# Bebra777228/PolGen-RVC

Hardware: AMD Instinct MI355X
Metric: real-time-factor (audio-sec/wall-sec) per GPU, 30s@16kHz RMVPE->48kHz (higher is better)
Workload: dtype f32 (conv products as 3 fp16 MFMAs of a hi/lo split, fp32 accumulate; fp32 elsewhere)

## Files before the change

include/rvcx.h:

```cpp
#ifndef RVCX_H
#define RVCX_H
#include <stdint.h>

#ifdef __cplusplus
extern "C" {
#endif

typedef struct rvcx_ctx rvcx_ctx;

typedef struct {
  const char* name;
  const void* data;
  int32_t dtype;
  int32_t ndim;
  int64_t shape[4];
} rvcx_tensor;

typedef struct {
  int32_t inter_channels, hidden_channels, filter_channels, n_heads, n_layers, kernel_size;
  int32_t n_resblocks;
  int32_t res_kernels[4];
  int32_t res_dilations[4][3];
  int32_t n_ups;
  int32_t up_rates[6], up_kernels[6];
// ... 364 lines not shown
                      int32_t* coarse, float* f0);
int rvcx_op_conv1d(rvcx_ctx*, const float* x, const float* w, const float* bias, const float* res,
                   float* y, int B, int Cin, int Tin, int Cout, int K, int stride, int dil,
                   int pad_left, int Tout, int groups, int pre_lrelu, float pre_slope, int act,
                   float act_slope, const int32_t* lens_in, const int32_t* lens_out);
int rvcx_op_resblock_pair(rvcx_ctx*, const float* x, const float* w1, const float* b1, const float* w2,
                          const float* b2, float* y, int B, int C, int T, int K, int dil, float slope, int fused,
                          const int32_t* lens);
int rvcx_op_resblock3(rvcx_ctx*, const float* x, const float* w1, const float* b1, const float* w2, const float* b2,
                      float* y, int B, int C, int T, const int32_t* dils, float slope, const int32_t* lens);
int rvcx_bench_resblock_pair(rvcx_ctx*, int B, int C, int T, int K, int dil, int fused, int iters,
                             float* ms_per_launch);
int rvcx_bench_conv1d(rvcx_ctx*, int B, int Cin, int Tin, int Cout, int K, int stride, int dil, int groups,
                      int iters, float* ms_per_launch);
int rvcx_conv_override(int tile, int variant, int splitk);
int rvcx_fx_stretch_override(int chunk_frames, int segment_frames);
int rvcx_op_convtranspose1d(rvcx_ctx*, const float* x, const float* w, const float* bias, float* y,
                            int B, int Cin, int Tin, int Cout, int K, int stride, int pad,
                            int pre_lrelu, float pre_slope);
int rvcx_op_conv2d3x3(rvcx_ctx*, const float* x, const float* w, const float* bias, const float* res,
                      float* y, int B, int Cin, int H, int W, int Cout, int act);
int rvcx_op_convblock2d(rvcx_ctx*, const float* x, const float* w1, const float* b1, const float* w2, const float* b2,
                        const float* wsc, const float* bsc, float* y, int B, int Cin, int Cout, int H, int W,
                        const int32_t* rows);
int rvcx_op_convtranspose2d(rvcx_ctx*, const float* x, const float* w, const float* bias, float* y,
                            int B, int Cin, int H, int W, int Cout, int act);
int rvcx_op_attention(rvcx_ctx*, const float* q, const float* k, const float* v, float* out, int B,
                      int H, int D, int T, float scale, const float* emb_rel_k,
                      const float* emb_rel_v, int window, const int32_t* lens);
int rvcx_op_gemm_tm(rvcx_ctx*, const float* x_cf, const float* w, const float* bias, const float* res_tm, int B, int T,
// ... 39 lines not shown
```

polgen-rvc_amd/_lib.py:

```python
from __future__ import annotations

import ctypes as C
import os
import threading
import types
from typing import Optional, Sequence

import numpy as np

_HERE = os.path.dirname(os.path.abspath(__file__))
LIB_PATH = os.environ.get("RVCX_LIBRARY") or os.path.join(_HERE, "librvcx.so")


class RvcxError(RuntimeError):
    pass


class Tensor(C.Structure):
    _fields_ = [("name", C.c_char_p), ("data", C.c_void_p), ("dtype", C.c_int32),
                ("ndim", C.c_int32), ("shape", C.c_int64 * 4)]


class SynthCfg(C.Structure):
    _fields_ = [("inter_channels", C.c_int32), ("hidden_channels", C.c_int32),
# ... 98 lines not shown
    k = min(Lx, Lb)
    fin = np.sin(0.5 * np.pi * np.arange(Lx) / max(Lx - 1, 1)) ** 2
    out[:k] = y[d:d + k] * fin[:k] + b[:k] * (1.0 - fin[:k])
    return out, y[d + Lb:d + Lb + Lx].copy(), d, scores, mags


_lib = None

SYMBOLS = [
    "rvcx_create", "rvcx_destroy", "rvcx_last_error", "rvcx_version", "rvcx_load_hubert",
    "rvcx_load_rmvpe", "rvcx_index_exhaustive", "rvcx_load_crepe", "rvcx_crepe_frames", "rvcx_crepe_predict", "rvcx_op_crepe_decode", "rvcx_get_f0_crepe_x", "rvcx_load_fcpe", "rvcx_fcpe_f0", "rvcx_fcpe_frames", "rvcx_get_f0_fcpe_x", "rvcx_op_fcpe_post", "rvcx_load_synth", "rvcx_unload_synth", "rvcx_load_index", "rvcx_load_index_ivf",
    "rvcx_weights_regions", "rvcx_weights_adopt", "rvcx_weights_clone", "rvcx_rmvpe_f0", "rvcx_rmvpe_frames", "rvcx_rmvpe_mel", "rvcx_synth_infer_taps", "rvcx_hubert_features",
    "rvcx_hubert_frames", "rvcx_synth_infer", "rvcx_synth_infer_window", "rvcx_synth_dec_rf", "rvcx_synth_upp", "rvcx_index_blend",
    "rvcx_out_len", "rvcx_convert_batch", "rvcx_convert_batch_f64", "rvcx_micro_batch", "rvcx_bucket_length", "rvcx_last_micro_batches", "rvcx_last_cuts", "rvcx_noise_len",
    "rvcx_get_f0", "rvcx_get_f0_x", "rvcx_vc", "rvcx_vc_frames", "rvcx_last_timing",
    "rvcx_flop_counter", "rvcx_fp32_reruns", "rvcx_mem_info", "rvcx_conv_profile", "rvcx_conv_profile_csv", "rvcx_stream", "rvcx_op_conv1d", "rvcx_op_resblock_pair", "rvcx_bench_resblock_pair", "rvcx_bench_conv1d", "rvcx_conv_override", "rvcx_op_convtranspose1d",
    "rvcx_op_conv2d3x3", "rvcx_op_convblock2d", "rvcx_op_convtranspose2d", "rvcx_op_attention", "rvcx_op_layernorm_c",
    "rvcx_op_bigru", "rvcx_op_highpass", "rvcx_highpass_exact", "rvcx_convert_batch_ex", "rvcx_get_f0_x_ex", "rvcx_fp32_layers", "rvcx_fp32_pinned",
    "rvcx_gru_fallbacks", "rvcx_gru_publish_probe", "rvcx_debug_inject", "rvcx_f0_file_track", "rvcx_op_gemm_tm", "rvcx_op_layernorm_tm",
    "rvcx_resample_len", "rvcx_resample_f64", "rvcx_resample_f64_kind", "rvcx_bench_gemm", "rvcx_device_info",
    "rvcx_convert_submit", "rvcx_convert_wait", "rvcx_convert_poll", "rvcx_convert_inflight", "rvcx_ticket_lead_ms",
    "rvcx_synth_infer_head", "rvcx_op_sola", "rvcx_stream_open", "rvcx_stream_step", "rvcx_stream_reset", "rvcx_stream_close",
    "rvcx_stream_out_len", "rvcx_stream_noise_len", "rvcx_stream_frames",
    "rvcx_stream_open_io", "rvcx_stream_in_len", "rvcx_stream_delays", "rvcx_stream_resample_delay", "rvcx_stream_last_taps",
    "rvcx_stream_set", "rvcx_op_stream_resample",
    "rvcx_stream_open_fx", "rvcx_stream_out_channels", "rvcx_stream_set_fx", "rvcx_stream_last_fx_ms", "rvcx_op_stream_fx",
    "rvcx_fx_reverb_host",
    "rvcx_fx_chain", "rvcx_op_fx_highpass", "rvcx_op_fx_compressor", "rvcx_op_fx_gate", "rvcx_op_fx_reverb", "rvcx_op_fx_shelf",
    "rvcx_op_fx_chorus", "rvcx_op_fx_mix", "rvcx_fx_chunk", "rvcx_fx_last_passes", "rvcx_fx_cte", "rvcx_fx_delay",
    "rvcx_fx_coeffs", "rvcx_fx_highpass_host", "rvcx_fx_biquad_host", "rvcx_fx_follower_host", "rvcx_fx_compressor_host",
    "rvcx_fx_gate_host", "rvcx_fx_comb_host", "rvcx_fx_allpass_host", "rvcx_fx_chorus_host", "rvcx_fx_mix_host",
# ... 1029 lines not shown
        self._ck(lib().rvcx_op_resblock3(self._h, _p(x), _p(w1), _p(b1), _p(w2), _p(b2), _p(y), B, Cc, T, _p(d, C.c_int32),
                                         C.c_float(slope), _p(li, C.c_int32)), "op_resblock3")
        return y

    def bench_resblock_pair(self, B, Cc, T, K, dil=1, fused=True, iters=10):
        ms = C.c_float(0)
        self._ck(lib().rvcx_bench_resblock_pair(self._h, B, Cc, T, K, dil, 1 if fused else 0, iters, C.byref(ms)),
                 "bench_resblock_pair")
        return ms.value, 4.0 * B * Cc * Cc * K * T / (ms.value * 1e-3) / 1e12

    @staticmethod
    def conv_override(tile=-1, variant=-1, splitk=-1):
        if lib().rvcx_conv_override(tile, variant, splitk) != 0:
            raise RvcxError("conv_override: " + (lib().rvcx_last_error(None) or b"").decode())

    def bench_conv1d(self, B, Cin, Tin, Cout, K, stride=1, dil=1, groups=1, iters=10):
        ms = C.c_float(0)
        self._ck(lib().rvcx_bench_conv1d(self._h, B, Cin, Tin, Cout, K, stride, dil, groups, iters, C.byref(ms)),
                 "bench_conv1d")
        pad = (K * dil - dil) // 2
        Tout = (Tin + 2 * pad - dil * (K - 1) - 1) // stride + 1
        flops = 2.0 * B * Cout * Tout * K * (Cin // groups)
        return ms.value, flops / (ms.value * 1e-3) / 1e12

    def convtranspose1d(self, x, w, bias=None, stride=1, pad=0, pre_lrelu=None):
        x, w = f32(x), f32(w)
        B, Cin, Tin = x.shape
        _, Cout, K = w.shape
        Tout = (Tin - 1) * stride - 2 * pad + K
        y = np.empty((B, Cout, Tout), np.float32)
# ... 1065 lines not shown
```

polgen-rvc_amd/csrc/api_ops.hip:

```cpp
#include "api_internal.h"
#include "h3_device.h"

using namespace rvcx;
using namespace rvcx::api;

static void to_host(Ctx& c, float* h, const float* d, size_t n) {
  RVCX_HIP(hipMemcpyAsync(h, d, n * sizeof(float), hipMemcpyDeviceToHost, c.stream));
  RVCX_HIP(hipStreamSynchronize(c.stream));
}
#define TEMP_REGION(C) WeightRegion tmp_region_; RegionScope tmp_scope_(*(C), tmp_region_)

extern "C" {

int rvcx_op_conv1d(rvcx_ctx* ctx, const float* x, const float* w, const float* bias, const float* res,
                   float* y, int B, int Cin, int Tin, int Cout, int K, int stride, int dil,
                   int pad_left, int Tout, int groups, int pre_lrelu, float pre_slope, int act,
                   float act_slope, const int32_t* lens_in, const int32_t* lens_out) {
  API_BEGIN(ctx)
  TEMP_REGION(C);
  size_t nx = (size_t)B * Cin * Tin, ny = (size_t)B * Cout * Tout;
  C->arena.reserve((nx + 2 * ny) * 4 + (64 << 20));
  C->arena.reset();
  ConvW L = make_conv(*C, w, bias, Cout, Cin / groups, K, groups, true);
  float* dx = to_dev(*C, x, nx);
// ... 219 lines not shown
  *ms_per_launch = ms / iters;
  (void)hipEventDestroy(e0);
  (void)hipEventDestroy(e1);
  C->arena.reset();
  API_END
}

int rvcx_conv_override(int tile, int variant, int splitk) {
  REQUIRE_DEBUG(nullptr, "rvcx_conv_override")
  rvcx::g_conv_override.tile = tile;
  rvcx::g_conv_override.variant = variant;
  rvcx::g_conv_override.splitk = splitk;
  return 0;
}

int rvcx_bench_conv1d(rvcx_ctx* ctx, int B, int Cin, int Tin, int Cout, int K, int stride, int dil, int groups,
                      int iters, float* ms_per_launch) {
  REQUIRE_DEBUG(ctx, "rvcx_bench_conv1d")
  API_BEGIN(ctx)
  TEMP_REGION(C);
  const int pad = (K * dil - dil) / 2;
  const int Tout = (Tin + 2 * pad - dil * (K - 1) - 1) / stride + 1;
  size_t nx = (size_t)B * Cin * Tin, ny = (size_t)B * Cout * Tout;
  C->arena.reserve((nx + 2 * ny) * 4 + (64 << 20));
  C->arena.reset();
  std::vector<float> w((size_t)Cout * (Cin / groups) * K), bias((size_t)Cout, 0.1f);
  for (size_t i = 0; i < w.size(); ++i) w[i] = (float)((i * 2654435761u) % 2001) / 1000.f - 1.f;
  ConvW L = make_conv(*C, w.data(), bias.data(), Cout, Cin / groups, K, groups, true);
  float* dx = C->arena.alloc<float>(nx);
  float* dy = C->arena.alloc<float>(ny);
// ... 652 lines not shown
```

polgen-rvc_amd/csrc/conv.h:

```cpp
#pragma once
#include "common.h"

namespace rvcx {

enum Act { ACT_NONE = 0, ACT_LRELU = 1, ACT_RELU = 2, ACT_GELU = 3, ACT_TANH = 4, ACT_SIGMOID = 5 };
enum OutMode { OUT_NORMAL = 0, OUT_SHUF1D = 1, OUT_SHUF2D = 2, OUT_TRANSPOSED = 3 };
enum Acc2 { ACC2_NONE = 0, ACC2_SET = 1, ACC2_ADD = 2, ACC2_ADD_DIV = 3 };

struct ConvArgs {
  const float* x = nullptr;
  const float* w = nullptr;
  const void* w_h3 = nullptr;
  const void* x_split = nullptr;
  void* y_split = nullptr;
  const float* bias = nullptr;
  const float* res = nullptr;
  float* y = nullptr;
  float* y2 = nullptr;
  const int* lens_in = nullptr;
  const int* lens_out = nullptr;
  int B = 1;
  int Cin_g = 0, Cin_gp = 0, Cout_g = 0, Cout_gp = 0, groups = 1;
  int Tin = 0;
  int Nout = 0;
// ... 102 lines not shown
struct ConvProfile {
  static constexpr int kMaxTiles = 72;
  long launches[kMaxTiles] = {0};
  double flops[kMaxTiles] = {0};
  double ms[kMaxTiles] = {0};
  int bm[kMaxTiles] = {0}, bn[kMaxTiles] = {0}, halo[kMaxTiles] = {0};
};
void conv_profile_begin();
void conv_profile_end(ConvProfile* out);
const char* conv_profile_csv();
void conv_init();
void launch_conv(ConvArgs a, hipStream_t stream);
int launch_conv_fast(ConvArgs& a, hipStream_t stream);
void conv_fast_describe(ConvProfile* p);
int launch_conv_h3(ConvArgs& a, int halo, int off_min, hipStream_t stream);
bool convt_thin_ok(const ConvArgs& a);
void launch_convt_thin(const ConvArgs& a, hipStream_t stream);
void convt_thin_init();
constexpr int kConvtThinSlot = 61;
bool conv3_thin_ok(const ConvArgs& a);
void launch_conv3_thin(const ConvArgs& a, hipStream_t stream);
constexpr int kConv3ThinSlot = 59;
bool conv_deep_ok(const ConvArgs& a);
void launch_conv_deep(const ConvArgs& a, hipStream_t stream);
constexpr int kConvDeepSlot = 63;
bool conv_h3_enabled();
bool conv_h3_configured();
bool conv_h3_split_ok(const ConvArgs& a);
void launch_splitk_finish(const ConvArgs& a, hipStream_t stream);
void conv_h3_describe(ConvProfile* p);
// ... 20 lines not shown
```

polgen-rvc_amd/csrc/conv.hip:

```cpp
#include "conv.h"
#include "conv_device.h"
#include "gemm.h"

#include <algorithm>
#include <cmath>

namespace rvcx {

template <int BM, int BN, int WR, int WC>
__global__ __launch_bounds__(256) void conv_mfma_kernel(const ConvArgs a) {
  constexpr int WM = BM / (32 * WR), WN = BN / (32 * WC);
  static_assert(WR * WC == 4 && WM >= 1 && WN >= 1, "bad tile");
  extern __shared__ float smem[];
  float* As = smem;
  float* Bs = smem + a.kk_chunk * a.ci_chunk * BM;

  const int tid = threadIdx.x, lane = tid & 63, wave = tid >> 6;
  const int wr = wave / WC, wc = wave % WC;
  const int i = lane & 31, h = lane >> 5;
  const int b = blockIdx.z;
  const int mt_per_g = (a.Cout_gp + BM - 1) / BM;
  const int g = blockIdx.y / mt_per_g, mt = blockIdx.y % mt_per_g;
  const int co0 = mt * BM;
  const int n0 = blockIdx.x * BN;
// ... 136 lines not shown
namespace {
struct ProfRec {
  hipEvent_t a, b;
  int tile;
  double flops;
  int cin, cout, k, nout, stride, B;
};
bool g_prof_on = false;
std::vector<ProfRec> g_prof;
}

void conv_profile_begin() {
  g_prof.clear();
  g_prof_on = true;
}

static std::string g_prof_csv;
const char* conv_profile_csv() { return g_prof_csv.c_str(); }

void conv_profile_end(ConvProfile* out) {
  g_prof_on = false;
  g_prof_csv = "tile,B,cin,cout,k,stride,nout,gflop,ms,tflops\n";
  for (int t = 0; t < kNumTiles; ++t) {
    out->bm[t] = kTiles[t].bm;
    out->bn[t] = kTiles[t].bn;
    out->halo[t] = -1;
  }
  conv_fast_describe(out);
  conv_h3_describe(out);
  resblock_pair_describe(out);
// ... 175 lines not shown
```

polgen-rvc_amd/csrc/conv_fast.hip:

```cpp
#include <cmath>
#include <cstdlib>

#include "conv.h"
#include "conv_device.h"

#ifdef RVCX_ABLATION
#define RVCX_DBG(a, bit) ((a).dbg & (bit))
#else
#define RVCX_DBG(a, bit) 0
#endif

namespace rvcx {

struct BufRsrc {
#if defined(__HIP_DEVICE_COMPILE__)
  __amdgpu_buffer_rsrc_t r;
#endif
};
constexpr int kBufOob = 0x7ffffff0;
__device__ __forceinline__ BufRsrc make_rsrc(const float* base, int bytes) {
  BufRsrc b;
#if defined(__HIP_DEVICE_COMPILE__)
  b.r = __builtin_amdgcn_make_buffer_rsrc(const_cast<float*>(base), 0, bytes, 0x00020000);
#endif
// ... 450 lines not shown
  p->bn[kConvDeepSlot] = 320;
  p->halo[kConvDeepSlot] = 300003;
  for (int t = 0; t < kNumFast; ++t) {
    const int s = 8 + t;
    p->bm[s] = kFast[t].bm;
    p->bn[s] = kFast[t].bn;
    p->halo[s] = kFast[t].cic == 32 ? 100000 : (kFast[t].halo < 0 ? 200000 : kFast[t].halo * 10);
  }
}

void launch_splitk_finish(const ConvArgs& a, hipStream_t stream) {
  const long total = (long)a.B * a.Cout_g * a.Nout;
  const long work = (((long)a.Cout_g * a.Nout) & 3) == 0 ? cdiv64(total, 4) : total;
  hipLaunchKernelGGL(conv_splitk_finish_kernel, dim3((unsigned)std::min<long>(cdiv64(work, 256), 4096)), dim3(256), 0,
                     stream, a);
}

int launch_conv_fast(ConvArgs& a, hipStream_t stream) {
  if (a.Cin_g == 1 && a.groups == 1 && a.ksize <= kCin1MaxK && a.kw >= 1 && a.ksize % a.kw == 0) {
    hipLaunchKernelGGL(conv_cin1_kernel, dim3(cdiv(a.Nout, 256), cdiv(a.Cout_g, 16), a.B), dim3(256), 0, stream, a);
    RVCX_HIP(hipGetLastError());
    return 7;
  }
  if (convt_thin_ok(a)) {
    launch_convt_thin(a, stream);
    return kConvtThinSlot;
  }
  RVCX_CHECK(!a.nz_har || a.out_mode == OUT_SHUF1D, "conv: a fused noise conv needs a polyphase ConvTranspose1d launch");
  if (conv_cout1_ok(a)) {
    static const bool on = !getenv("RVCX_COUT1") || atoi(getenv("RVCX_COUT1")) != 0;
// ... 108 lines not shown
```

polgen-rvc_amd/csrc/conv_h3.hip:

```cpp
#include <algorithm>
#include <cmath>
#include <cstdlib>

#include "conv.h"
#include "conv_device.h"
#include "h3_device.h"

#ifdef RVCX_ABLATION
#define H3_DBG(a, bit) ((a).dbg & (bit))
#else
#define H3_DBG(a, bit) 0
#endif

namespace rvcx {

template <int BM, int BN, int WR, int WC, int KKT, int HALO, int STRIDE, bool LIN, bool XS = false>
__global__ __launch_bounds__(256, ((LIN && BM * BN >= 8192) || BN >= 512) ? 2 : 3) void conv_h3_kernel(const ConvArgs a) {
  constexpr int WM = BM / (32 * WR), WN = BN / (32 * WC);
  constexpr int WROW = LIN ? BN : BN * STRIDE + HALO;
  constexpr int NBTILE = LIN ? KKT : 1;
  constexpr int A_ELEMS = KKT * 2 * 2 * BM;
  constexpr int NA = (A_ELEMS + 255) / 256;
  constexpr int B_TASKS = NBTILE * 2 * WROW;
  constexpr int NBT = (B_TASKS + 255) / 256;
// ... 310 lines not shown
  if (a.groups != 1 || a.ksize == 1 || a.out_mode != OUT_NORMAL) return false;
  if (a.stride != 1 && !(a.stride == 2 && a.kw == a.ksize)) return false;
  if (a.Cin_g % 16 != 0 || a.Cout_g % 16 != 0 || a.Cin_g != a.Cin_gp) return false;
  {
    int lo = 1 << 30, hi = -(1 << 30);
    for (int kk = 0; kk < a.ksize; ++kk) {
      lo = std::min(lo, conv_tap_off(a, kk));
      hi = std::max(hi, conv_tap_off(a, kk));
    }
    if (hi - lo > 320) return false;
  }
  if ((long)a.Cin_gp * a.x_cs * 4 >= kH3Oob || (long)a.Cout_g * a.y_cs * 4 >= kH3Oob) return false;
  return true;
}

int launch_conv_h3(ConvArgs& a, int halo, int off_min, hipStream_t stream) {
  const bool split = a.x_split || a.y_split;
  RVCX_CHECK(!split || conv_h3_split_ok(a), "conv_h3: pre-split activations on a launch that cannot take them");
  if (!a.w_h3 || !conv_h3_enabled()) return -1;
  if (a.Cin_gp % 16 != 0 || (a.stride != 1 && !(a.stride == 2 && a.kw == a.ksize))) return -1;
  if (a.groups != 1 && (split || a.ksize == 1 || a.stride != 1 || a.out_mode != OUT_NORMAL || a.Cin_g != a.Cin_gp)) return -1;
  if ((long)a.Cin_gp * a.x_cs * 4 >= kH3Oob || (long)a.ksize * a.Cin_gp * a.Cout_gp * 4 >= kH3Oob) return -1;
  const bool lin = a.ksize == 1 && a.stride == 1;
  const int nchunk = a.Cin_gp / 16;
  const long cap_item = a.part_cap_item > 0 ? a.part_cap_item : a.part_cap;
  static const bool wide3x3 = getenv("RVCX_WIDE3X3") && atoi(getenv("RVCX_WIDE3X3")) != 0;
  auto select = [&](int Bsel, int forcedS, int* tile_out, int* s_out) {
    int best = -1, S = 1;
    double best_t = 1e300;
    for (int t = 0; t < kNumH3; ++t) {
      const H3Cfg& F = kH3[t];
// ... 24 lines not shown
    *tile_out = best;
    *s_out = S;
  };
  int best = -1, S = 1;
  select(1, 0, &best, &S);
  static const int tile2_mask = getenv("RVCX_TILE2_MASK") ? atoi(getenv("RVCX_TILE2_MASK")) : 255;
  const int cls = (a.out_mode != OUT_NORMAL) ? 8 : (lin ? 2 : (halo > 64 ? 1 : 4));
  int cls2 = cls;
  if (a.x_split || a.y_split) cls2 |= 16;
  const bool tile_for_batch = (tile2_mask & cls) && (!(cls2 & 16) || (tile2_mask & 16));
  if (best >= 0 && a.B > 1 && tile_for_batch) {
    int b2 = -1, s2 = 1;
    select(a.B, S, &b2, &s2);
    if (b2 >= 0 && s2 == S) best = b2;
  }
  if (best < 0) return -1;
  const H3Cfg& F = kH3[best];
  a.off_min = off_min;
  a.wrow = halo;
  a.splitk = S;
  {
    static int dbg = -1;
    if (dbg < 0) dbg = getenv("RVCX_CONV_DBG") ? atoi(getenv("RVCX_CONV_DBG")) : 0;
    a.dbg = dbg;
  }
  dim3 grid(cdiv(a.Nout, F.bn), cdiv(a.Cout_gp, F.bm), a.B * a.groups * S);
  {
    static const bool log = getenv("RVCX_CONV_LOG") != nullptr;
    if (log)
      fprintf(stderr, "h3 tile %d (%dx%d halo %d) S %d grid %u %u %u B %d Cin %d Cout %d k %d Nout %d xs %d ys %d\n", best,
// ... 11 lines not shown
```

polgen-rvc_amd/csrc/ctx.h:

```cpp
#pragma once
#include <memory>

#include "common.h"
#include "conv.h"
#include "gemm.h"

namespace rvcx {

struct SynthModel;
struct RmvpeModel;
struct FcpeModel;
struct CrepeModel;
struct HubertModel;
struct IndexData;

class WeightRegion {
 public:
  static constexpr size_t kChunkBytes = (size_t)32 << 20;
  static constexpr int kMaxFlags = 4096;
  static constexpr size_t kHeaderBytes = kMaxFlags;
  WeightRegion() {
    flags_.reset(new uint8_t[kMaxFlags]);
    std::memset(flags_.get(), 0, kMaxFlags);
  }
// ... 224 lines not shown
  }
  void gemm_on(GemmArgs a, hipStream_t s) {
    const double f = 2.0 * (double)a.rows * a.cout * a.cin;
    flops += f;
    a.ovf = dev_err;
    a.seq = ++launch_seq;
    {
      const int si = (s == stream2) ? 1 : (s == aux[0] ? 2 : (s == aux[1] ? 3 : 0));
      if (!splitk_buf[si]) RVCX_HIP(hipMalloc(&splitk_buf[si], kSplitKFloats * splitk_items * sizeof(float)));
      a.part = splitk_buf[si];
      a.part_cap = kSplitKFloats * splitk_items;
    }
    conv_launch_gemm(a, f, s);
  }
  void conv(const ConvArgs& a) { conv_on(a, stream); }
  void conv_on(ConvArgs a, hipStream_t s) {
    flops += conv_flops(a);
    const int si = (s == stream2) ? 1 : (s == aux[0] ? 2 : (s == aux[1] ? 3 : 0));
    if (!splitk_buf[si]) RVCX_HIP(hipMalloc(&splitk_buf[si], kSplitKFloats * splitk_items * sizeof(float)));
    a.part = splitk_buf[si];
    a.part_cap = kSplitKFloats * splitk_items;
    a.part_cap_item = kSplitKFloats;
    a.ovf = dev_err;
    a.seq = ++launch_seq;
    launch_conv(a, s);
  }
};

struct RegionScope {
  Ctx& c;
  WeightRegion* prev;
  RegionScope(Ctx& cc, WeightRegion& r) : c(cc), prev(cc.slab.cur_) { cc.slab.cur_ = &r; }
  ~RegionScope() { c.slab.cur_ = prev; }
};

struct ConvW {
  const float* w = nullptr;
// ... 56 lines not shown
```

polgen-rvc_amd/csrc/layers.h:

```cpp
#pragma once
#include "ctx.h"

namespace rvcx {

inline ConvArgs conv1d_args(const ConvW& w, const float* x, float* y, int B, int Tin, int Tout,
                            int stride = 1, int dil = 1, int pad = 0) {
  ConvArgs a;
  conv_set_weights(a, w);
  a.x = x;
  a.y = y;
  a.B = B;
  a.Tin = Tin;
  a.Nout = Tout;
  a.stride = stride;
  a.dil = dil;
  a.pad = pad;
  a.x_bs = (long)w.cin * Tin;
  a.x_cs = Tin;
  a.y_bs = (long)w.cout * Tout;
  a.y_cs = Tout;
  return a;
}

inline void conv_set_res(ConvArgs& a, const float* res, int C, int T) {
// ... 75 lines not shown
  a.rowpitch = Wp;
  a.dil = 1;
  a.pad = 0;
  a.stride = 1;
  a.x_bs = (long)L.w.cin * H * Wp;
  a.x_cs = H * Wp;
  a.y_bs = (long)L.cout_real * 2 * H * Wpo;
  a.y_cs = 2 * H * Wpo;
  a.out_mode = OUT_SHUF2D;
  a.sh_cout = L.cout_real;
  a.wp_in = Wp;
  a.wp_out = Wpo;
  return a;
}

ConvT1dW make_convT1d(Ctx& c, const float* w, const float* bias, int cin, int cout, int k, int s, int p);
ConvT2dW make_convT2d(Ctx& c, const float* w, const float* scale, const float* shift, int cin, int cout);

}
```

polgen-rvc_amd/csrc/synth.hip:

```cpp
#include <algorithm>
#include <cmath>
#include <cstdlib>

#include "models.h"
#include "ops.h"

namespace rvcx {

std::vector<float> wn_weight(const TensorTable& t, const std::string& p, int dim) {
  if (t.has(p + ".weight")) return t.f32(p + ".weight");
  std::string gn = p + ".parametrizations.weight.original0", vn = p + ".parametrizations.weight.original1";
  if (!t.has(gn)) {
    gn = p + ".weight_g";
    vn = p + ".weight_v";
  }
  std::vector<float> g = t.f32(gn), v = t.f32(vn);
  const auto shp = t.shape(vn);
  RVCX_CHECK(shp.size() == 3, "weight-norm tensor must be 3-D: " + p);
  const int64_t d0 = shp[0], d1 = shp[1], d2 = shp[2];
  std::vector<float> w(v.size());
  if (dim == 0) {
    RVCX_CHECK((int64_t)g.size() == d0, "weight_g shape: " + p);
    for (int64_t a = 0; a < d0; ++a) {
      double ss = 0.0;
// ... 317 lines not shown
    launch_copy_strided(z + head, z2, B * inter, Tk, T, Tk, s);
    std::swap(z, z2);
  }
  float* g = A.alloc<float>((size_t)B * gin);
  for (int b = 0; b < B; ++b)
    RVCX_HIP(hipMemcpyAsync(g + (size_t)b * gin, m.emb_g + (size_t)sidv[b] * gin, gin * sizeof(float),
                            hipMemcpyDeviceToDevice, s));
  {
    float* h = att;
    float* xin = qkv;
    float* acts = tmp;
    float* rs = hbuf;
    RVCX_CHECK(filt >= 2 * hid, "buffer reuse assumes filter_channels >= 2*hidden");
    float* wout = A.alloc<float>((size_t)B * hid * T);
    float* mbuf = A.alloc<float>((size_t)B * half * T);
    float* gc = A.alloc<float>((size_t)B * 6 * hid);
    for (int f = 3; f >= 0; --f) {
      const auto& F = m.flows[f];
      launch_flip_channels(z, z2, B, inter, Tk, s);
      std::swap(z, z2);
      ConvArgs a = conv1d_args(F.pre, z, h, B, Tk, Tk);
      a.x_bs = (long)inter * Tk;
      a.lens_out = lens;
      c.conv(a);
      a = conv1d_args(F.cond, g, gc, B, 1, 1);
      c.conv(a);
      for (int i = 0; i < 3; ++i) {
        a = conv1d_args(F.in_l[i], h, xin, B, Tk, Tk, 1, 1, (F.in_l[i].k - 1) / 2);
        a.lens_in = lens;
        a.lens_out = lens;
        c.conv(a);
        launch_wn_gate(xin, gc, i * 2 * hid, 6 * hid, acts, B, hid, Tk, s);
        a = conv1d_args(F.rs_l[i], acts, rs, B, Tk, Tk);
        a.lens_out = lens;
        c.conv(a);
        launch_wn_res_skip(h, wout, rs, B, hid, Tk, i == 2, i == 0, lens, s);
      }
      a = conv1d_args(F.post, wout, mbuf, B, Tk, Tk);
      a.lens_out = lens;
      c.conv(a);
      launch_coupling_sub(z, mbuf, B, half, Tk, lens, s);
    }
  }
  if (io.z_out)
    RVCX_HIP(hipMemcpyAsync(io.z_out, z, (size_t)B * inter * Tk * sizeof(float), hipMemcpyDeviceToDevice, s));
  tm.mark(2);
  if (io.ev_decoder) RVCX_HIP(hipEventRecord(io.ev_decoder, s));

  if (!c.serial) RVCX_HIP(hipStreamWaitEvent(s, c.ev_src[1], 0));
  static const int dec_batch_env = getenv("RVCX_DEC_BATCH") ? std::max(1, atoi(getenv("RVCX_DEC_BATCH"))) : 8;
  bool equal_lens = true;
  if (io.lens_host)
    for (int b = 1; b < B; ++b) equal_lens &= io.lens_host[b] == io.lens_host[0];
  const int dec_batch = equal_lens ? dec_batch_env : 1;
  const int C0 = cf.up_initial_channel;
// ... 203 lines not shown
```

Before: 1233.

## Fuse each flow coupling layer into a single LDS-resident kernel with halo

Adds a fused kernel that runs an entire residual-coupling flow layer (pre conv, three WN dilated convs with gating, res/skip convs, post conv and coupling subtraction) for a time window plus halo in LDS, using the hi/lo fp16 MFMA scheme. This replaces about 15 launches per flow and their global round trips with one launch per flow. The channel flip is folded into the indexing, and the cond convs for all four flows are hoisted ahead of the loop. The cost is recomputing halo columns and heavy LDS use, which may limit occupancy. The fused path is on by default when h3 is enabled, profiling is off and the shapes fit.

```diff
diff --git a/include/rvcx.h b/include/rvcx.h
--- a/include/rvcx.h
+++ b/include/rvcx.h
@@ -402,6 +402,8 @@
 int rvcx_bench_conv1d(rvcx_ctx*, int B, int Cin, int Tin, int Cout, int K, int stride, int dil, int groups,
                       int iters, float* ms_per_launch);
 int rvcx_conv_override(int tile, int variant, int splitk);
+int rvcx_flow_fuse_override(int mode, int width);
+int64_t rvcx_flow_fused_launches(void);
 int rvcx_fx_stretch_override(int chunk_frames, int segment_frames);
 int rvcx_op_convtranspose1d(rvcx_ctx*, const float* x, const float* w, const float* bias, float* y,
                             int B, int Cin, int Tin, int Cout, int K, int stride, int pad,
diff --git a/polgen-rvc_amd/_lib.py b/polgen-rvc_amd/_lib.py
--- a/polgen-rvc_amd/_lib.py
+++ b/polgen-rvc_amd/_lib.py
@@ -136,7 +136,7 @@
     "rvcx_hubert_frames", "rvcx_synth_infer", "rvcx_synth_infer_window", "rvcx_synth_dec_rf", "rvcx_synth_upp", "rvcx_index_blend",
     "rvcx_out_len", "rvcx_convert_batch", "rvcx_convert_batch_f64", "rvcx_micro_batch", "rvcx_bucket_length", "rvcx_last_micro_batches", "rvcx_last_cuts", "rvcx_noise_len",
     "rvcx_get_f0", "rvcx_get_f0_x", "rvcx_vc", "rvcx_vc_frames", "rvcx_last_timing",
-    "rvcx_flop_counter", "rvcx_fp32_reruns", "rvcx_mem_info", "rvcx_conv_profile", "rvcx_conv_profile_csv", "rvcx_stream", "rvcx_op_conv1d", "rvcx_op_resblock_pair", "rvcx_bench_resblock_pair", "rvcx_bench_conv1d", "rvcx_conv_override", "rvcx_op_convtranspose1d",
+    "rvcx_flop_counter", "rvcx_fp32_reruns", "rvcx_mem_info", "rvcx_conv_profile", "rvcx_conv_profile_csv", "rvcx_stream", "rvcx_op_conv1d", "rvcx_op_resblock_pair", "rvcx_bench_resblock_pair", "rvcx_bench_conv1d", "rvcx_conv_override", "rvcx_flow_fuse_override", "rvcx_flow_fused_launches", "rvcx_op_convtranspose1d",
     "rvcx_op_conv2d3x3", "rvcx_op_convblock2d", "rvcx_op_convtranspose2d", "rvcx_op_attention", "rvcx_op_layernorm_c",
     "rvcx_op_bigru", "rvcx_op_highpass", "rvcx_highpass_exact", "rvcx_convert_batch_ex", "rvcx_get_f0_x_ex", "rvcx_fp32_layers", "rvcx_fp32_pinned",
     "rvcx_gru_fallbacks", "rvcx_gru_publish_probe", "rvcx_debug_inject", "rvcx_f0_file_track", "rvcx_op_gemm_tm", "rvcx_op_layernorm_tm",
@@ -1196,6 +1196,17 @@
         if lib().rvcx_conv_override(tile, variant, splitk) != 0:
             raise RvcxError("conv_override: " + (lib().rvcx_last_error(None) or b"").decode())
 
+    @staticmethod
+    def flow_fuse_override(mode=-1, width=0):
+        if lib().rvcx_flow_fuse_override(int(mode), int(width)) != 0:
+            raise RvcxError("flow_fuse_override: " + (lib().rvcx_last_error(None) or b"").decode())
+
+    @staticmethod
+    def flow_fused_launches() -> int:
+        f = lib().rvcx_flow_fused_launches
+        f.restype = C.c_int64
+        return int(f())
+
     def bench_conv1d(self, B, Cin, Tin, Cout, K, stride=1, dil=1, groups=1, iters=10):
         ms = C.c_float(0)
         self._ck(lib().rvcx_bench_conv1d(self._h, B, Cin, Tin, Cout, K, stride, dil, groups, iters, C.byref(ms)),
diff --git a/polgen-rvc_amd/csrc/api_ops.hip b/polgen-rvc_amd/csrc/api_ops.hip
--- a/polgen-rvc_amd/csrc/api_ops.hip
+++ b/polgen-rvc_amd/csrc/api_ops.hip
@@ -257,6 +257,19 @@
   return 0;
 }
 
+int rvcx_flow_fuse_override(int mode, int width) {
+  REQUIRE_DEBUG(nullptr, "rvcx_flow_fuse_override")
+  if (mode < -1 || mode > 1 || (width != 0 && width != 16 && width != 32)) {
+    g_last_error = "rvcx_flow_fuse_override: mode in {-1, 0, 1}, width in {0, 16, 32}";
+    return -1;
+  }
+  rvcx::g_flow_fuse_override.mode = mode;
+  rvcx::g_flow_fuse_override.width = width;
+  return 0;
+}
+
+int64_t rvcx_flow_fused_launches(void) { return (int64_t)rvcx::g_flow_fused_launches.load(); }
+
 int rvcx_bench_conv1d(rvcx_ctx* ctx, int B, int Cin, int Tin, int Cout, int K, int stride, int dil, int groups,
                       int iters, float* ms_per_launch) {
   REQUIRE_DEBUG(ctx, "rvcx_bench_conv1d")
diff --git a/polgen-rvc_amd/csrc/conv.h b/polgen-rvc_amd/csrc/conv.h
--- a/polgen-rvc_amd/csrc/conv.h
+++ b/polgen-rvc_amd/csrc/conv.h
@@ -140,6 +140,9 @@
 int launch_conv_fast(ConvArgs& a, hipStream_t stream);
 void conv_fast_describe(ConvProfile* p);
 int launch_conv_h3(ConvArgs& a, int halo, int off_min, hipStream_t stream);
+int conv_h3_plan_splitk(const ConvArgs& a, int halo);
+int conv_h3_route_splitk(const ConvArgs& a);
+bool conv_profile_on();
 bool convt_thin_ok(const ConvArgs& a);
 void launch_convt_thin(const ConvArgs& a, hipStream_t stream);
 void convt_thin_init();
diff --git a/polgen-rvc_amd/csrc/conv.hip b/polgen-rvc_amd/csrc/conv.hip
--- a/polgen-rvc_amd/csrc/conv.hip
+++ b/polgen-rvc_amd/csrc/conv.hip
@@ -174,6 +174,8 @@
   g_prof.clear();
   g_prof_on = true;
 }
+
+bool conv_profile_on() { return g_prof_on; }
 
 static std::string g_prof_csv;
 const char* conv_profile_csv() { return g_prof_csv.c_str(); }
diff --git a/polgen-rvc_amd/csrc/conv_fast.hip b/polgen-rvc_amd/csrc/conv_fast.hip
--- a/polgen-rvc_amd/csrc/conv_fast.hip
+++ b/polgen-rvc_amd/csrc/conv_fast.hip
@@ -488,6 +488,20 @@
   const long work = (((long)a.Cout_g * a.Nout) & 3) == 0 ? cdiv64(total, 4) : total;
   hipLaunchKernelGGL(conv_splitk_finish_kernel, dim3((unsigned)std::min<long>(cdiv64(work, 256), 4096)), dim3(256), 0,
                      stream, a);
+}
+
+int conv_h3_route_splitk(const ConvArgs& a) {
+  if (a.Cin_g == 1 || a.groups != 1 || a.stride != 1 || a.out_mode != OUT_NORMAL || a.Cin_gp % 16 != 0) return -1;
+  if (a.x_split || a.y_split || a.nz_har) return -1;
+  if (convt_thin_ok(a) || conv_cout1_ok(a)) return -1;
+  if ((long)a.Cin_gp * a.x_cs * 4 >= kBufOob || (long)a.ksize * a.Cin_gp * a.Cout_gp * 4 >= kBufOob) return -1;
+  int off_min = 1 << 30, off_max = -(1 << 30);
+  for (int kk = 0; kk < a.ksize; ++kk) {
+    off_min = std::min(off_min, conv_tap_off(a, kk));
+    off_max = std::max(off_max, conv_tap_off(a, kk));
+  }
+  if (conv3_thin_ok(a) || conv_deep_ok(a)) return -1;
+  return conv_h3_plan_splitk(a, off_max - off_min);
 }
 
 int launch_conv_fast(ConvArgs& a, hipStream_t stream) {
diff --git a/polgen-rvc_amd/csrc/conv_h3.hip b/polgen-rvc_amd/csrc/conv_h3.hip
--- a/polgen-rvc_amd/csrc/conv_h3.hip
+++ b/polgen-rvc_amd/csrc/conv_h3.hip
@@ -348,7 +348,7 @@
   return true;
 }
 
-int launch_conv_h3(ConvArgs& a, int halo, int off_min, hipStream_t stream) {
+static int h3_choose(const ConvArgs& a, int halo, int* S_out) {
   const bool split = a.x_split || a.y_split;
   RVCX_CHECK(!split || conv_h3_split_ok(a), "conv_h3: pre-split activations on a launch that cannot take them");
   if (!a.w_h3 || !conv_h3_enabled()) return -1;
@@ -403,6 +403,18 @@
     select(a.B, S, &b2, &s2);
     if (b2 >= 0 && s2 == S) best = b2;
   }
+  *S_out = S;
+  return best;
+}
+
+int conv_h3_plan_splitk(const ConvArgs& a, int halo) {
+  int S = 1;
+  return h3_choose(a, halo, &S) < 0 ? -1 : S;
+}
+
+int launch_conv_h3(ConvArgs& a, int halo, int off_min, hipStream_t stream) {
+  int S = 1;
+  const int best = h3_choose(a, halo, &S);
   if (best < 0) return -1;
   const H3Cfg& F = kH3[best];
   a.off_min = off_min;
diff --git a/polgen-rvc_amd/csrc/ctx.h b/polgen-rvc_amd/csrc/ctx.h
--- a/polgen-rvc_amd/csrc/ctx.h
+++ b/polgen-rvc_amd/csrc/ctx.h
@@ -262,13 +262,16 @@
     conv_launch_gemm(a, f, s);
   }
   void conv(const ConvArgs& a) { conv_on(a, stream); }
-  void conv_on(ConvArgs a, hipStream_t s) {
-    flops += conv_flops(a);
+  void offer_splitk(ConvArgs& a, hipStream_t s) {
     const int si = (s == stream2) ? 1 : (s == aux[0] ? 2 : (s == aux[1] ? 3 : 0));
     if (!splitk_buf[si]) RVCX_HIP(hipMalloc(&splitk_buf[si], kSplitKFloats * splitk_items * sizeof(float)));
     a.part = splitk_buf[si];
     a.part_cap = kSplitKFloats * splitk_items;
     a.part_cap_item = kSplitKFloats;
+  }
+  void conv_on(ConvArgs a, hipStream_t s) {
+    flops += conv_flops(a);
+    offer_splitk(a, s);
     a.ovf = dev_err;
     a.seq = ++launch_seq;
     launch_conv(a, s);
diff --git a/polgen-rvc_amd/csrc/flow_fused.hip b/polgen-rvc_amd/csrc/flow_fused.hip
--- /dev/null
+++ b/polgen-rvc_amd/csrc/flow_fused.hip
@@ -0,0 +1,317 @@
+#include <algorithm>
+#include <atomic>
+#include <cstdlib>
+
+#include "conv.h"
+#include "conv_device.h"
+#include "h3_device.h"
+#include "layers.h"
+
+namespace rvcx {
+
+FlowFuseOverride g_flow_fuse_override;
+std::atomic<long> g_flow_fused_launches{0};
+
+namespace {
+
+constexpr int kFlowLdsMax = 160 * 1024;
+
+template <int U, bool LIN>
+__device__ __forceinline__ void flow_mma(f32x16& acc, const H3Rsrc& wr, int cout_gp, int nchunk, int co, int h,
+                                         const uint4* Bs, int wrow, int col, int cb0, int cb1) {
+  const int slab = 4 * cout_gp * 16, aoff = (h * cout_gp + co) * 16, opoff = 2 * cout_gp * 16;
+  const int nunit = LIN ? (cb1 - cb0 + U - 1) / U : cb1 - cb0;
+  uint4 cur[U][2], nxt[U][2];
+#pragma unroll
+  for (int j = 0; j < U; ++j) {
+    const int ch = LIN ? cb0 + j : cb0, kk = LIN ? 0 : j;
+    const bool ok = ch < cb1;
+    const int off = (kk * nchunk + ch) * slab + aoff;
+    cur[j][0] = h3_load4(wr, ok ? off : kH3Oob);
+    cur[j][1] = h3_load4(wr, ok ? off + opoff : kH3Oob);
+  }
+  for (int u = 0; u < nunit; ++u) {
+#pragma unroll
+    for (int j = 0; j < U; ++j) {
+      const int ch = LIN ? cb0 + (u + 1) * U + j : cb0 + u + 1, kk = LIN ? 0 : j;
+      const bool ok = ch < cb1;
+      const int off = (kk * nchunk + ch) * slab + aoff;
+      nxt[j][0] = h3_load4(wr, ok ? off : kH3Oob);
+      nxt[j][1] = h3_load4(wr, ok ? off + opoff : kH3Oob);
+    }
+#pragma unroll
+    for (int j = 0; j < U; ++j) {
+      const int ch = LIN ? cb0 + u * U + j : cb0 + u;
+      if (!LIN || ch < cb1) {
+        const int bi = (ch * 4 + h) * wrow + col + (LIN ? 0 : j);
+        const half8 a0 = __builtin_bit_cast(half8, cur[j][0]), a2 = __builtin_bit_cast(half8, cur[j][1]);
+        const half8 a1 = a0 * (_Float16)(1.f / kH3Scale);
+        const half8 b0 = __builtin_bit_cast(half8, Bs[bi]), b1 = __builtin_bit_cast(half8, Bs[bi + 2 * wrow]);
+        acc = h3_mfma(a0, b0, acc);
+        acc = h3_mfma(a1, b1, acc);
+        acc = h3_mfma(a2, b0, acc);
+      }
+    }
+#pragma unroll
+    for (int j = 0; j < U; ++j) {
+      cur[j][0] = nxt[j][0];
+      cur[j][1] = nxt[j][1];
+    }
+  }
+}
+
+__device__ __forceinline__ float flow_gate(float ta, float sa) {
+  float v = tanhf(ta) * (1.f / (1.f + expf(-sa)));
+  asm volatile("" : "+v"(v));
+  return v;
+}
+
+__device__ __forceinline__ float bias_at(const FlowConv& cv, int row) { return row < cv.cout ? cv.bias[row] : 0.f; }
+
+template <int U, bool LIN>
+__device__ __forceinline__ void flow_block(f32x16& v, const FlowConv& cv, int co0, int i, int h, const uint4* Bs, int wrow,
+                                           int col) {
+  const H3Rsrc wr = h3_rsrc(cv.w, cv.k * cv.nchunk * 4 * cv.cout_gp * 16);
+  constexpr float inv = 1.f / kH3Scale;
+  const int rb = co0 + 4 * h;
+  if (cv.S == 1) {
+    f32x16 acc;
+#pragma unroll
+    for (int r = 0; r < 16; ++r) acc[r] = 0.f;
+    flow_mma<U, LIN>(acc, wr, cv.cout_gp, cv.nchunk, co0 + i, h, Bs, wrow, col, 0, cv.nchunk);
+#pragma unroll
+    for (int r = 0; r < 16; ++r) acc[r] *= inv;
+#pragma unroll
+    for (int r = 0; r < 16; ++r) v[r] = (acc[r] + bias_at(cv, rb + (r & 3) + 8 * (r >> 2))) + 0.f;
+  } else {
+    f32x16 tot;
+#pragma unroll
+    for (int r = 0; r < 16; ++r) tot[r] = 0.f;
+    for (int ks = 0; ks < cv.S; ++ks) {
+      f32x16 acc;
+#pragma unroll
+      for (int r = 0; r < 16; ++r) acc[r] = 0.f;
+      flow_mma<U, LIN>(acc, wr, cv.cout_gp, cv.nchunk, co0 + i, h, Bs, wrow, col, ks * cv.nchunk / cv.S,
+                       (ks + 1) * cv.nchunk / cv.S);
+#pragma unroll
+      for (int r = 0; r < 16; ++r) acc[r] *= inv;
+#pragma unroll
+      for (int r = 0; r < 16; ++r) tot[r] += acc[r];
+    }
+#pragma unroll
+    for (int r = 0; r < 16; ++r) v[r] = tot[r] + bias_at(cv, rb + (r & 3) + 8 * (r >> 2));
+  }
+}
+
+template <int K>
+__global__ __launch_bounds__(512) void flow_layer_kernel(const FlowLayerArgs a) {
+  extern __shared__ uint4 flow_lds[];
+  const int tid = threadIdx.x, nthr = blockDim.x, lane = tid & 63, wave = tid >> 6, nw = nthr >> 6;
+  const int i = lane & 31, h = lane >> 5;
+  const int b = blockIdx.y, w0 = blockIdx.x * a.W, g0 = w0 - a.R;
+  const int NB = a.NB, hid = a.hid, half = a.half, T = a.T, nbn = NB / 32;
+  const int len = a.lens ? a.lens[b] : T;
+  float* zb = a.z + (long)b * a.bs;
+  const int x1row = a.flip ? half - 1 : half, x1step = a.flip ? -1 : 1;
+  if (w0 >= len) {
+    const int nc = min(a.W, T - w0);
+    for (int t = tid; t < half * nc; t += nthr) {
+      const int c = t / nc, p = t - c * nc;
+      zb[(long)(x1row + x1step * c) * T + w0 + p] = 0.f;
+    }
+    return;
+  }
+  const int rpre = a.cv[0].nchunk * 16, rmax = max(hid, rpre), wrow = NB + 2 * a.pmax;
+  float* Hf = reinterpret_cast<float*>(flow_lds);
+  float* Wo = Hf + hid * NB;
+  uint4* As = reinterpret_cast<uint4*>(Wo + rmax * NB);
+  uint4* Hs = As + rmax / 4 * NB;
+  unsigned ovf = 0;
+
+  auto split = [&](const float* src, int nch, uint4* dst, int wr_, int poff, int bit) {
+    for (int t = tid; t < nch * 2 * wr_; t += nthr) {
+      const int ch2 = t / wr_, q = t - ch2 * wr_, p = q - poff;
+      half8 hi, lo;
+      const bool in = p >= 0 && p < NB;
+      const int tt = g0 + p;
+      const bool own = in && tt >= w0 && tt < w0 + a.W && tt < T;
+#pragma unroll
+      for (int c = 0; c < 8; ++c) {
+        const float v = in ? src[(ch2 * 8 + c) * NB + p] : 0.f;
+        if (own && !(fabsf(v) < kH3ActLimit)) ovf |= 1u << bit;
+        const _Float16 vh = (_Float16)v;
+        hi[c] = vh;
+        lo[c] = (_Float16)((v - (float)vh) * kH3Scale);
+      }
+      dst[((ch2 >> 1) * 4 + (ch2 & 1)) * wr_ + q] = __builtin_bit_cast(uint4, hi);
+      dst[((ch2 >> 1) * 4 + 2 + (ch2 & 1)) * wr_ + q] = __builtin_bit_cast(uint4, lo);
+    }
+  };
+
+  for (int t = tid; t < rpre * NB; t += nthr) {
+    const int r = t / NB, p = t - r * NB, tt = g0 + p;
+    const int row = a.flip ? a.inter - 1 - r : r;
+    Wo[t] = (r < half && tt >= 0 && tt < T) ? zb[(long)row * T + tt] : 0.f;
+  }
+  __syncthreads();
+  split(Wo, a.cv[0].nchunk, As, NB, 0, 0);
+  __syncthreads();
+  for (int it = wave; it < (hid / 32) * nbn; it += nw) {
+    const int m = it / nbn, p = (it - m * nbn) * 32 + i, tt = g0 + p;
+    const bool live = tt >= 0 && tt < len;
+    f32x16 v;
+    flow_block<4, true>(v, a.cv[0], m * 32, i, h, As, NB, p);
+#pragma unroll
+    for (int r = 0; r < 16; ++r) Hf[(m * 32 + 4 * h + (r & 3) + 8 * (r >> 2)) * NB + p] = live ? v[r] : 0.f;
+  }
+  __syncthreads();
+  const float* gcb = a.gc + (long)b * a.gstride;
+  for (int l = 0; l < 3; ++l) {
+    const FlowConv& ci = a.cv[1 + 2 * l];
+    const FlowConv& cr = a.cv[2 + 2 * l];
+    split(Hf, hid / 16, Hs, wrow, a.pmax, 1 + 2 * l);
+    __syncthreads();
+    for (int it = wave; it < (hid / 32) * nbn; it += nw) {
+      const int m = it / nbn, p = (it - m * nbn) * 32 + i, tt = g0 + p;
+      const bool live = tt >= 0 && tt < len;
+      const bool own = tt >= w0 && tt < w0 + a.W && tt < T;
+      const int col = p + a.pmax - (K - 1) / 2;
+      f32x16 va, vb;
+      flow_block<K, false>(va, ci, m * 32, i, h, Hs, wrow, col);
+      flow_block<K, false>(vb, ci, hid + m * 32, i, h, Hs, wrow, col);
+      const float* ga = gcb + l * 2 * hid + m * 32 + 4 * h;
+      typedef _Float16 half4 __attribute__((ext_vector_type(4)));
+#pragma unroll
+      for (int g = 0; g < 4; ++g) {
+        half4 hi, lo;
+#pragma unroll
+        for (int q = 0; q < 4; ++q) {
+          const int r = 4 * g + q;
+          const float ta = (live ? va[r] : 0.f) + ga[8 * g + q];
+          const float sa = (live ? vb[r] : 0.f) + ga[hid + 8 * g + q];
+          const float v = flow_gate(ta, sa);
+          if (own && !(fabsf(v) < kH3ActLimit)) ovf |= 1u << (2 + 2 * l);
+          const _Float16 vh = (_Float16)v;
+          hi[q] = vh;
+          lo[q] = (_Float16)((v - (float)vh) * kH3Scale);
+        }
+        const int e = ((m * 2 + (g >> 1)) * 4 + (g & 1)) * NB + p;
+        char* base = reinterpret_cast<char*>(As);
+        *reinterpret_cast<half4*>(base + (long)e * 16 + 8 * h) = hi;
+        *reinterpret_cast<half4*>(base + (long)(e + 2 * NB) * 16 + 8 * h) = lo;
+      }
+    }
+    __syncthreads();
+    const bool first = l == 0, last = l == 2;
+    for (int it = wave; it < (cr.cout_gp / 32) * nbn; it += nw) {
+      const int m = it / nbn, p = (it - m * nbn) * 32 + i, tt = g0 + p;
+      const bool live = tt >= 0 && tt < len;
+      f32x16 v;
+      flow_block<4, true>(v, cr, m * 32, i, h, As, NB, p);
+      const bool skip = last || m * 32 >= hid;
+      const int row0 = (skip && !last ? m * 32 - hid : m * 32) + 4 * h;
+#pragma unroll
+      for (int r = 0; r < 16; ++r) {
+        const int e = (row0 + (r & 3) + 8 * (r >> 2)) * NB + p;
+        const float y = live ? v[r] : 0.f;
+        if (!skip) {
+          Hf[e] = live ? Hf[e] + y : 0.f;
+        } else {
+          const float o = first ? y : Wo[e] + y;
+          Wo[e] = last ? (live ? o : 0.f) : o;
+        }
+      }
+    }
+    __syncthreads();
+  }
+  const FlowConv& cp = a.cv[7];
+  split(Wo, hid / 16, As, NB, 0, 7);
+  __syncthreads();
+  for (int it = wave; it < (cp.cout_gp / 32) * nbn; it += nw) {
+    const int m = it / nbn, p = (it - m * nbn) * 32 + i, tt = g0 + p;
+    const bool live = tt >= 0 && tt < len;
+    const bool own = tt >= w0 && tt < w0 + a.W && tt < T;
+    f32x16 v;
+    flow_block<4, true>(v, cp, m * 32, i, h, As, NB, p);
+#pragma unroll
+    for (int r = 0; r < 16; ++r) {
+      const int c = m * 32 + 4 * h + (r & 3) + 8 * (r >> 2);
+      if (own && c < half) {
+        float* px = zb + (long)(x1row + x1step * c) * T + tt;
+        const float mv = live ? v[r] : 0.f;
+        float o = *px - mv;
+        if (tt >= len) o = 0.f;
+        *px = o;
+      }
+    }
+  }
+#pragma unroll
+  for (int j = 0; j < 8; ++j)
+    if (ovf & (1u << j)) report_h3_overflow(a.ovf, a.cv[j].word, a.seq0 + j);
+}
+
+void (*flow_kernel(int k))(const FlowLayerArgs) {
+  return k == 3 ? flow_layer_kernel<3> : (k == 5 ? flow_layer_kernel<5> : (k == 7 ? flow_layer_kernel<7> : nullptr));
+}
+
+}
+
+int flow_layer_lds_bytes(int hid, int rpre, int NB, int pmax) {
+  const int rmax = std::max(hid, rpre);
+  return (hid * NB + 2 * rmax * NB + hid * (NB + 2 * pmax)) * 4;
+}
+
+bool flow_layer_shape_ok(FlowLayerArgs& a, int width) {
+  if (a.hid % 32 != 0 || a.hid <= 0 || a.half <= 0 || a.inter != 2 * a.half) return false;
+  const int k = a.cv[1].k;
+  if (!flow_kernel(k) || a.cv[3].k != k || a.cv[5].k != k) return false;
+  a.pmax = (k - 1) / 2;
+  a.R = 3 * a.pmax;
+  for (int j = 0; j < 8; ++j) {
+    const FlowConv& c = a.cv[j];
+    const bool in_l = j == 1 || j == 3 || j == 5;
+    if (!c.w || !c.bias || c.cout_gp % 32 != 0 || c.nchunk < 1) return false;
+    if (!in_l && (c.k != 1 || c.S != 1)) return false;
+    if (c.S < 1 || c.nchunk / c.S < 1) return false;
+    if (j > 0 && c.nchunk * 16 != a.hid) return false;
+    if ((long)c.k * c.nchunk * 4 * c.cout_gp * 16 >= kH3Oob) return false;
+  }
+  if (a.cv[0].cout_gp != a.hid || a.cv[0].nchunk * 16 < a.half) return false;
+  if (a.cv[1].cout_gp != 2 * a.hid || a.cv[3].cout_gp != 2 * a.hid || a.cv[5].cout_gp != 2 * a.hid) return false;
+  if (a.cv[2].cout_gp != 2 * a.hid || a.cv[4].cout_gp != 2 * a.hid || a.cv[6].cout_gp != a.hid) return false;
+  if (a.cv[7].cout_gp < a.half) return false;
+  for (int W : {32, 16}) {
+    if (width != 0 && W != width) continue;
+    const int NB = (W + 2 * a.R + 31) / 32 * 32;
+    if (flow_layer_lds_bytes(a.hid, a.cv[0].nchunk * 16, NB, a.pmax) > kFlowLdsMax) continue;
+    a.W = W;
+    a.NB = NB;
+    return true;
+  }
+  return false;
+}
+
+void launch_flow_layer(const FlowLayerArgs& a, hipStream_t stream) {
+  auto kern = flow_kernel(a.cv[1].k);
+  RVCX_CHECK(kern && a.W > 0 && a.NB >= a.W + 2 * a.R, "flow_layer: unplanned launch");
+  const int lds = flow_layer_lds_bytes(a.hid, a.cv[0].nchunk * 16, a.NB, a.pmax);
+  static bool raised[8] = {false};
+  if (!raised[a.cv[1].k]) {
+    RVCX_HIP(hipFuncSetAttribute(reinterpret_cast<const void*>(kern), hipFuncAttributeMaxDynamicSharedMemorySize, kFlowLdsMax));
+    raised[a.cv[1].k] = true;
+  }
+  const int items = a.hid / 32 * (a.NB / 32);
+  int nw = 4, waste = 1 << 30;
+  for (int w = 4; w <= 8; ++w) {
+    const int ws = (items + w - 1) / w * w - items;
+    if (ws <= waste) {
+      waste = ws;
+      nw = w;
+    }
+  }
+  hipLaunchKernelGGL(kern, dim3(cdiv(a.T, a.W), a.B), dim3(nw * 64), lds, stream, a);
+  ++g_flow_fused_launches;
+  RVCX_HIP(hipGetLastError());
+}
+
+}
diff --git a/polgen-rvc_amd/csrc/layers.h b/polgen-rvc_amd/csrc/layers.h
--- a/polgen-rvc_amd/csrc/layers.h
+++ b/polgen-rvc_amd/csrc/layers.h
@@ -1,4 +1,6 @@
 #pragma once
+#include <atomic>
+
 #include "ctx.h"
 
 namespace rvcx {
@@ -113,6 +115,31 @@
   return a;
 }
 
+struct FlowConv {
+  const void* w = nullptr;
+  const float* bias = nullptr;
+  int* word = nullptr;
+  int cout = 0, cout_gp = 0, nchunk = 0, k = 1, S = 1;
+};
+struct FlowLayerArgs {
+  float* z = nullptr;
+  long bs = 0;
+  int B = 1, inter = 0, half = 0, hid = 0, T = 0;
+  int flip = 0;
+  const int* lens = nullptr;
+  const float* gc = nullptr;
+  int gstride = 0;
+  FlowConv cv[8];
+  int W = 0, NB = 0, R = 0, pmax = 0;
+  int* ovf = nullptr;
+  int seq0 = 0;
+};
+bool flow_layer_shape_ok(FlowLayerArgs& a, int width);
+void launch_flow_layer(const FlowLayerArgs& a, hipStream_t stream);
+struct FlowFuseOverride { int mode = -1, width = 0; };
+extern FlowFuseOverride g_flow_fuse_override;
+extern std::atomic<long> g_flow_fused_launches;
+
 ConvT1dW make_convT1d(Ctx& c, const float* w, const float* bias, int cin, int cout, int k, int s, int p);
 ConvT2dW make_convT2d(Ctx& c, const float* w, const float* scale, const float* shift, int cin, int cout);
 
diff --git a/polgen-rvc_amd/csrc/synth.hip b/polgen-rvc_amd/csrc/synth.hip
--- a/polgen-rvc_amd/csrc/synth.hip
+++ b/polgen-rvc_amd/csrc/synth.hip
@@ -355,31 +355,86 @@
     RVCX_CHECK(filt >= 2 * hid, "buffer reuse assumes filter_channels >= 2*hidden");
     float* wout = A.alloc<float>((size_t)B * hid * T);
     float* mbuf = A.alloc<float>((size_t)B * half * T);
-    float* gc = A.alloc<float>((size_t)B * 6 * hid);
+    float* gc_all = A.alloc<float>((size_t)4 * B * 6 * hid);
+    for (int f = 3; f >= 0; --f) {
+      ConvArgs a = conv1d_args(m.flows[f].cond, g, gc_all + (size_t)f * B * 6 * hid, B, 1, 1);
+      c.conv(a);
+    }
+    auto flow_conv = [&](const SynthModel::Flow& F, int j) {
+      ConvArgs a;
+      if (j == 0) {
+        a = conv1d_args(F.pre, z, h, B, Tk, Tk);
+        a.x_bs = (long)inter * Tk;
+      } else if (j == 7) {
+        a = conv1d_args(F.post, wout, mbuf, B, Tk, Tk);
+      } else if (j & 1) {
+        const ConvW& w = F.in_l[(j - 1) / 2];
+        a = conv1d_args(w, h, xin, B, Tk, Tk, 1, 1, (w.k - 1) / 2);
+        a.lens_in = lens;
+      } else {
+        a = conv1d_args(F.rs_l[(j - 2) / 2], acts, rs, B, Tk, Tk);
+      }
+      a.lens_out = lens;
+      return a;
+    };
+    static const bool fuse_env = !getenv("RVCX_FLOW_FUSE") || atoi(getenv("RVCX_FLOW_FUSE")) != 0;
+    static const int width_env = getenv("RVCX_FLOW_W") ? atoi(getenv("RVCX_FLOW_W")) : 0;
+    bool fuse = (g_flow_fuse_override.mode < 0 ? fuse_env : g_flow_fuse_override.mode != 0) && conv_h3_enabled() &&
+                !conv_profile_on() && head == 0 && inter == 2 * half;
+    FlowLayerArgs fa[4];
+    for (int f = 3; f >= 0 && fuse; --f) {
+      const auto& F = m.flows[f];
+      FlowLayerArgs& L = fa[f];
+      L.z = z;
+      L.bs = (long)inter * Tk;
+      L.B = B;
+      L.inter = inter;
+      L.half = half;
+      L.hid = hid;
+      L.T = Tk;
+      L.flip = (f & 1);
+      L.lens = lens;
+      L.gc = gc_all + (size_t)f * B * 6 * hid;
+      L.gstride = 6 * hid;
+      for (int j = 0; j < 8 && fuse; ++j) {
+        ConvArgs a = flow_conv(F, j);
+        c.offer_splitk(a, s);
+        const int S = conv_h3_route_splitk(a);
+        FlowConv& v = L.cv[j];
+        v.w = a.w_h3;
+        v.bias = a.bias;
+        v.word = a.ovf_layer;
+        v.cout = a.Cout_g;
+        v.cout_gp = a.Cout_gp;
+        v.nchunk = a.Cin_gp / 16;
+        v.k = a.ksize;
+        v.S = S;
+        fuse = S >= 1 && a.Cin_g == (j == 0 ? half : hid);
+      }
+      fuse = fuse && F.cond.cout == 6 * hid &&
+             flow_layer_shape_ok(L, g_flow_fuse_override.width ? g_flow_fuse_override.width : width_env);
+    }
     for (int f = 3; f >= 0; --f) {
       const auto& F = m.flows[f];
+      if (fuse) {
+        for (int j = 0; j < 8; ++j) c.flops += conv_flops(flow_conv(F, j));
+        fa[f].ovf = c.dev_err;
+        fa[f].seq0 = c.launch_seq + 1;
+        c.launch_seq += 8;
+        launch_flow_layer(fa[f], s);
+        continue;
+      }
+      const float* gc = gc_all + (size_t)f * B * 6 * hid;
       launch_flip_channels(z, z2, B, inter, Tk, s);
       std::swap(z, z2);
-      ConvArgs a = conv1d_args(F.pre, z, h, B, Tk, Tk);
-      a.x_bs = (long)inter * Tk;
-      a.lens_out = lens;
-      c.conv(a);
-      a = conv1d_args(F.cond, g, gc, B, 1, 1);
-      c.conv(a);
+      c.conv(flow_conv(F, 0));
       for (int i = 0; i < 3; ++i) {
-        a = conv1d_args(F.in_l[i], h, xin, B, Tk, Tk, 1, 1, (F.in_l[i].k - 1) / 2);
-        a.lens_in = lens;
-        a.lens_out = lens;
-        c.conv(a);
+        c.conv(flow_conv(F, 1 + 2 * i));
         launch_wn_gate(xin, gc, i * 2 * hid, 6 * hid, acts, B, hid, Tk, s);
-        a = conv1d_args(F.rs_l[i], acts, rs, B, Tk, Tk);
-        a.lens_out = lens;
-        c.conv(a);
+        c.conv(flow_conv(F, 2 + 2 * i));
         launch_wn_res_skip(h, wout, rs, B, hid, Tk, i == 2, i == 0, lens, s);
       }
-      a = conv1d_args(F.post, wout, mbuf, B, Tk, Tk);
-      a.lens_out = lens;
-      c.conv(a);
+      c.conv(flow_conv(F, 7));
       launch_coupling_sub(z, mbuf, B, half, Tk, lens, s);
     }
   }
```

Result: no change. 1242, median of 6 (+0.7%).
